# Gregor-Mendel-Institute/SNPmatch

Hardware: AMD Instinct MI355X
Metric: accession×SNP comparisons/sec (whole node); achieved HBM GB/s vs peak (higher is better)
Workload: dtype f64

## Files before the change

### snpmatch_amd/csrc/snpm_api.hip

```cpp
#include "snpmatch_hip.h"

#include <hip/hip_runtime.h>

#include <fcntl.h>
#include <unistd.h>

#include <algorithm>
#include <atomic>
#include <cerrno>
#include <cmath>
#include <cstdarg>
#include <cstdio>
#include <cstdlib>
#include <chrono>
#include <cstring>
#include <map>
#include <mutex>
#include <new>
#include <stdexcept>
#include <string>
#include <thread>
#include <vector>

#include "snpm_kernels.hpp"
// ... 148 lines not shown
    int64_t ld = 0;
    int packed = 0;
    int8_t *d = nullptr;
    int *d_other = nullptr;
    hipEvent_t uploaded = nullptr;
    bool upload_pending = false;
    hipEvent_t used = nullptr;
    bool used_valid = false;
    uint8_t *dT = nullptr;
    int64_t pitchT = 0;
    int dT_state = 0;
    std::vector<snpm_query *> queries;
};

constexpr int REEVAL_CAP = 64;

struct snpm_query {
    snpm_panel *panel = nullptr;
    int64_t n = 0, row0 = 0;
    int64_t *d_row_idx = nullptr;
    double *d_w = nullptr;
    double *d_lut = nullptr;
    int lut_skip = -1;
    double *d_score = nullptr;
    int64_t *d_ninfo = nullptr;
    double *own_score = nullptr;
    int64_t *own_ninfo = nullptr;
    double wsum = 0;
    bool all_integer = false;
    bool hard01 = false;
    uint8_t *d_wbits = nullptr;
    void *d_cert = nullptr;
    int64_t eref_chunk = -1, eref_after = -1;
    bool count_valid = false;
    bool cert_count_clean = false;
    std::vector<snpm_ctx::Cached> owned;
    const char *last_kernel = "";
    int reeval_path = 0;
    bool transient_panel = false;
    double *cert_eref() const { return (double *)d_cert; }
    int *cert_count() const { return (int *)((char *)d_cert + 8); }
    int32_t *cert_cols() const { return (int32_t *)((char *)d_cert + 16); }
};

struct snpm_carry {
    snpm_ctx *ctx = nullptr;
    int64_t n_acc = 0, ld = 0;
    double *d_score = nullptr;
    int64_t *d_ninfo = nullptr;
    double *d_E = nullptr;
    int32_t *d_cols = nullptr;
    int *d_ncols = nullptr;
    int64_t n_cols = -1;
    int64_t n_rows = 0, n_slabs = 0;
    long double wsum = 0;
    int mode = -1;
    bool all_integer = true;
    bool finished = false;
    double *own_score = nullptr;
    int64_t *own_ninfo = nullptr;
    int64_t len = 0;
};

namespace {

int set_err(snpm_ctx *ctx, int code, const char *fmt, ...)
// ... 236 lines not shown
    if (const char *s = getenv("SNPM_SHARED_TILES")) ctx->shared_force_tiles = std::max(0, atoi(s));
    if (const char *s = getenv("SNPM_KIN_WS_MB")) ctx->kin_ws_bytes = (size_t)std::max(1, atoi(s)) << 20;
    if (const char *s = getenv("SNPM_SITE_WS_MB")) ctx->site_ws_bytes = (size_t)std::max(1, atoi(s)) << 20;
    if (const char *s = getenv("SNPM_LD_WS_MB")) ctx->ld_ws_bytes = (size_t)std::max(1, atoi(s)) << 20;
    if (const char *s = getenv("SNPM_WIN_WS_MB")) ctx->win_ws_bytes = (size_t)std::max(1, atoi(s)) << 20;
    if (const char *s = getenv("SNPM_F1X_WS_MB")) ctx->f1x_ws_bytes = (size_t)std::max(1, atoi(s)) << 20;
    if (const char *s = getenv("SNPM_PAR_WS_MB")) ctx->par_ws_bytes = (size_t)std::max(1, atoi(s)) << 20;
    if (const char *s = getenv("SNPM_SIM_WS_MB")) ctx->sim_ws_bytes = (size_t)std::max(1, atoi(s)) << 20;
    if (const char *s = getenv("SNPM_MOS_WS_MB")) ctx->mos_ws_bytes = (size_t)std::max(1, atoi(s)) << 20;
    if (const char *s = getenv("SNPM_IBD_WS_MB")) ctx->ibd_ws_bytes = (size_t)std::max(1, atoi(s)) << 20;
    if (const char *s = getenv("SNPM_IBD_BITS_MB")) ctx->ibd_bits_bytes = (size_t)std::max(1, atoi(s)) << 20;
    if (const char *s = getenv("SNPM_MK_WS_MB")) ctx->mk_ws_bytes = (size_t)std::max(1, atoi(s)) << 20;
    ctx->stage_threads = default_stage_threads();
    if (const char *s = getenv("SNPM_STAGE_THREADS")) ctx->stage_threads = std::max(1, atoi(s));
    if (const char *s = getenv("SNPM_STAGE_MB")) ctx->ld_want = (size_t)std::max(1, atoi(s)) << 20;
    if (const char *s = getenv("SNPM_HOST_PACK")) ctx->host_pack = atoi(s);
    if (const char *s = getenv("SNPM_ODIRECT")) ctx->odirect = atoi(s);
    if (getenv("SNPM_NO_AVX2")) ctx->ld_avx2 = 0;
    ctx->ld_nt = (cpu_has_avx2() && ctx->ld_avx2 && !getenv("SNPM_NO_NT")) ? 1 : 0;
    *out = ctx;
    return SNPM_OK;
} SNPM_GUARD(nullptr)

static void orphan_query(snpm_query *q, bool use_hip)
{
    snpm_ctx *ctx = q->panel ? q->panel->ctx : nullptr;
    if (use_hip && ctx) {
        while (!q->owned.empty()) query_release(q, q->owned.back().p);
    } else {
        q->owned.clear();
    }
    q->d_row_idx = nullptr; q->d_w = nullptr; q->d_lut = nullptr; q->d_score = nullptr; q->d_ninfo = nullptr;
    q->own_score = nullptr; q->own_ninfo = nullptr; q->d_wbits = nullptr; q->d_cert = nullptr;
    q->panel = nullptr;
}

static void orphan_panel(snpm_panel *p, bool use_hip)
{
    for (snpm_query *q : p->queries) orphan_query(q, use_hip);
    p->queries.clear();
    if (use_hip) {
        if (p->d) (void)hipFree(p->d);
        if (p->dT) (void)hipFree(p->dT);
        if (p->uploaded) (void)hipEventDestroy(p->uploaded);
        if (p->used) (void)hipEventDestroy(p->used);
    }
    if (p->ctx && p->ctx->last_touched == p) p->ctx->last_touched = nullptr;
    p->used = nullptr;
    p->used_valid = false;
    p->d = nullptr;
    p->d_other = nullptr;
    p->dT = nullptr;
    p->uploaded = nullptr;
    p->ctx = nullptr;
}

int snpm_destroy(snpm_ctx *ctx)
{
    if (!ctx) return SNPM_OK;
    const bool use_hip = hip_alive();
    if (use_hip) {
        (void)hipSetDevice(ctx->device);
        (void)hipDeviceSynchronize();
    }
    for (snpm_group *g : ctx->groups) group_forget_ctx(g, ctx, use_hip);
    ctx->groups.clear();
// ... 144 lines not shown
```

### snpmatch_amd/csrc/snpm_api_carry.hpp

```cpp
int snpm_carry_create(snpm_ctx *ctx, int64_t n_acc, snpm_carry **out)
try {
    if (!ctx) return SNPM_ERR_BADARG;
    CHECK_ARG(ctx, out != nullptr && n_acc >= 1, "carry needs n_acc >= 1");
    HIPCHK(ctx, hipSetDevice(ctx->device));
    snpm_carry *c = new snpm_carry();
    c->ctx = ctx;
    c->n_acc = n_acc;
    c->ld = ((n_acc + 255) / 256) * 256;
    hipError_t e = hipMalloc((void **)&c->own_score, (size_t)c->ld * sizeof(double));
    if (e == hipSuccess) e = hipMalloc((void **)&c->own_ninfo, (size_t)c->ld * sizeof(int64_t));
    if (e == hipSuccess) e = hipMalloc((void **)&c->d_E, 256 + REEVAL_CAP * sizeof(int32_t));
    c->d_score = c->own_score;
    c->d_ninfo = c->own_ninfo;
    c->len = c->ld;
    if (e != hipSuccess) {
        if (c->own_score) (void)hipFree(c->own_score);
        if (c->own_ninfo) (void)hipFree(c->own_ninfo);
        delete c;
        return set_err(ctx, SNPM_ERR_OOM, "carry allocation failed: %s", hipGetErrorString(e));
    }
    c->d_ncols = (int *)((char *)c->d_E + 8);
    c->d_cols = (int32_t *)((char *)c->d_E + 256);
    ctx->carries.push_back(c);
    *out = c;
// ... 34 lines not shown
    }
    delete c;
    return SNPM_OK;
}

int snpm_carry_bind_outputs(snpm_carry *c, void *d_score, void *d_ninfo)
{
    CHECK_CARRY(c);
    snpm_ctx *ctx = c->ctx;
    CHECK_ARG(ctx, (d_score == nullptr) == (d_ninfo == nullptr), "bind both outputs or neither");
    CHECK_ARG(ctx, c->n_slabs == 0, "bind the outputs before the first slab");
    c->d_score = d_score ? (double *)d_score : c->own_score;
    c->d_ninfo = d_ninfo ? (int64_t *)d_ninfo : c->own_ninfo;
    c->len = d_score ? c->n_acc : c->ld;
    return snpm_carry_reset(c);
}

int snpm_carry_set_columns(snpm_carry *c, const int32_t *cols, int64_t ncols)
{
    CHECK_CARRY(c);
    snpm_ctx *ctx = c->ctx;
    CHECK_ARG(ctx, c->n_slabs == 0, "set the column list before the first slab");
    CHECK_ARG(ctx, ncols >= 1 && ncols <= REEVAL_CAP && cols, "a column list holds 1..64 accessions (more: a strict pass over all of them)");
    for (int64_t i = 0; i < ncols; ++i) CHECK_ARG(ctx, cols[i] >= 0 && cols[i] < c->n_acc, "accession index outside the panel");
    HIPCHK(ctx, hipSetDevice(ctx->device));
    const int nc = (int)ncols;
    HIPCHK(ctx, hipMemcpyAsync(c->d_cols, cols, (size_t)ncols * sizeof(int32_t), hipMemcpyHostToDevice, ctx->stream));
    HIPCHK(ctx, hipMemcpyAsync(c->d_ncols, &nc, sizeof(int), hipMemcpyHostToDevice, ctx->stream));
    HIPCHK(ctx, hipStreamSynchronize(ctx->stream));
    c->n_cols = ncols;
    return SNPM_OK;
}

int snpm_query_run_carry(snpm_query *q, int64_t chunk, int skip_hets, int mode, int64_t chunks_after, snpm_carry *c)
try {
    CHECK_QUERY(q);
    CHECK_CARRY(c);
    snpm_ctx *ctx = q->panel->ctx;
    snpm_panel *p = q->panel;
    CHECK_ARG(ctx, c->ctx == ctx && c->n_acc == p->n_acc, "the carry belongs to another context or panel width");
    CHECK_ARG(ctx, chunk >= 1 && chunks_after >= 0, "chunk must be >= 1 and chunks_after >= 0");
    CHECK_ARG(ctx, mode == SNPM_MODE_EXACT || mode == SNPM_MODE_STRICT || mode == SNPM_MODE_FAST, "unknown mode");
    CHECK_ARG(ctx, !c->finished, "the carry was finished: reset it first");
    CHECK_ARG(ctx, c->mode < 0 || c->mode == mode, "every slab of a job is scored in the same mode");
    CHECK_ARG(ctx, chunks_after == 0 || q->n % chunk == 0, "every slab but the last must hold a multiple of `chunk` rows");
    CHECK_ARG(ctx, c->n_cols < 0 || mode == SNPM_MODE_STRICT, "a column-list carry takes strict slabs");
    HIPCHK(ctx, hipSetDevice(ctx->device));
    int rc = wait_upload(p);
    if (rc) return rc;
    const int skip = skip_hets ? 1 : 0;
    q->transient_panel = true;
    q->count_valid = false;
    if (c->n_cols >= 0) {
        rc = run_strict_sparse(q, skip, chunk, c->d_cols, c->d_ncols, c->d_score);
        if (rc) return rc;
        HIPCHK(ctx, hipMemcpyAsync(c->d_score, ctx->ws_tmp_score.p, (size_t)c->n_cols * sizeof(double),
                                   hipMemcpyDeviceToDevice, ctx->stream));
    } else if (mode == SNPM_MODE_STRICT) {
        q->last_kernel = "k_strict4";
        rc = run_strict_chain(q, skip, chunk, nullptr, c->d_score, c->d_ninfo, c->d_score, c->d_ninfo);
        if (rc) return rc;
    } else {
        Certify cert;
        cert.on = (mode == SNPM_MODE_EXACT);
        cert.flag = false;
        cert.chunk = chunk;
        cert.chunks_after = chunks_after;
        FastGeom g;
        rc = run_fast(q, skip, &g, cert);
        if (rc) return rc;
        const bool bounded = cert.on && q->n > 0;
        if (bounded && q->all_integer) {
            rc = ensure_eref(q, chunk, chunks_after);
            if (rc) return rc;
        }
        hipLaunchKernelGGL(k_carry_add, dim3((unsigned)((p->n_acc + 255) / 256)), dim3(256), 0, ctx->stream, c->d_score,
                           c->d_ninfo, (const double *)q->d_score, (const int64_t *)q->d_ninfo, p->n_acc, c->d_E,
                           bounded ? (const double *)q->cert_eref() : (const double *)nullptr,
                           (bounded && !q->all_integer) ? efast_bound(q, g) : 0.0);
        HIPCHK(ctx, hipGetLastError());
        c->all_integer = c->all_integer && (q->all_integer || q->n == 0);
    }
    c->mode = mode;
    c->n_rows += q->n;
    c->n_slabs += 1;
    c->wsum += q->wsum;
    return SNPM_OK;
} SNPM_GUARD(((q && q->panel) ? q->panel->ctx : nullptr))

static bool carry_is_exact(const snpm_carry *c) { return c->all_integer && c->wsum < 9.0e15L; }

static double carry_e_extra(const snpm_carry *c)
{
    const double u = 1.1102230246251565e-16;
    const double m = (double)(c->n_slabs + 1);
    return (double)(c->wsum * (long double)(m * u / (1.0 - m * u))) * 1.0000001;
}

int snpm_carry_error_bound(snpm_carry *c, double *bound)
{
    CHECK_CARRY(c);
    snpm_ctx *ctx = c->ctx;
    CHECK_ARG(ctx, bound != nullptr, "bound is NULL");
    *bound = 0.0;
    if (c->mode != SNPM_MODE_EXACT || carry_is_exact(c)) return SNPM_OK;
    HIPCHK(ctx, hipSetDevice(ctx->device));
    int rc = ensure_pinned(ctx, 64);
    if (rc) return rc;
    HIPCHK(ctx, hipMemcpyAsync(ctx->h_pinned, c->d_E, sizeof(double), hipMemcpyDeviceToHost, ctx->stream));
    HIPCHK(ctx, hipStreamSynchronize(ctx->stream));
    *bound = *(const double *)ctx->h_pinned + carry_e_extra(c);
// ... 57 lines not shown
```

### snpmatch_amd/csrc/snpm_api_cert.hpp

```cpp
int ensure_pinned(snpm_ctx *ctx, size_t bytes)
{
    if (ctx->h_pinned_cap >= bytes) return SNPM_OK;
    if (ctx->h_pinned) {
        HIPCHK(ctx, hipStreamSynchronize(ctx->stream));
        (void)hipHostFree(ctx->h_pinned);
    }
    ctx->h_pinned = nullptr;
    ctx->h_pinned_cap = 0;
    const size_t want = std::max<size_t>(bytes, 64 << 10);
    HIPCHK(ctx, hipHostMalloc(&ctx->h_pinned, want, hipHostMallocDefault));
    ctx->h_pinned_cap = want;
    return SNPM_OK;
}

int ensure_eref(snpm_query *q, int64_t chunk, int64_t chunks_after)
{
    snpm_ctx *ctx = q->panel->ctx;
    if (q->eref_chunk == chunk && q->eref_after == chunks_after) return SNPM_OK;
    const int64_t K = (q->n + chunk - 1) / chunk;
    const int grid = (int)std::max<int64_t>(1, std::min<int64_t>(K, 2048));
    int rc = ensure(ctx, ctx->ws_epart, (size_t)grid * sizeof(double));
    if (rc) return rc;
    hipLaunchKernelGGL(k_eref, dim3((unsigned)grid), dim3(256), 0, ctx->stream, (const double *)q->d_w, q->n, chunk,
                       chunks_after, (double *)ctx->ws_epart.p);
    hipLaunchKernelGGL(k_efinish, dim3(1), dim3(256), 0, ctx->stream, (const double *)ctx->ws_epart.p, grid, q->n, chunk,
                       chunks_after, q->cert_eref());
    HIPCHK(ctx, hipGetLastError());
    q->eref_chunk = chunk;
    q->eref_after = chunks_after;
    return SNPM_OK;
}

double efast_bound(const snpm_query *q, const FastGeom &g)
{
    const double u = 1.1102230246251565e-16;
    const int64_t epoch_adds = (int64_t)EPOCH_TILES * (g.packed ? TILE_ROWS : std::max(g.tile_rows, TILE_ROWS));
    const double m = (double)(std::min<int64_t>(g.part_rows, epoch_adds) + REDUCE_GROUP + g.n_groups + 2);
    return (q->wsum * (m * u / (1.0 - m * u))) * 1.0000001;
}

struct Certify {
    bool on = false;
    bool flag = true;
    int64_t chunk = 1000, chunks_after = 0;
};

int fast_tile_rows(const snpm_query *q, bool bits)
{
    const snpm_panel *p = q->panel;
    if (p->packed) return bits ? BITS_TILE_ROWS : Q4_TILE_ROWS * Q4_RUN;
    const bool long_tiles = q->n >= p->ctx->long_scan_rows && p->n_acc > 2 * WAVE * 4;
    return long_tiles ? LONG_TILE_ROWS : TILE_ROWS;
}

int run_fast(snpm_query *q, int skip, FastGeom *geom_out, const Certify &cert)
{
    snpm_ctx *ctx = q->panel->ctx;
    snpm_panel *p = q->panel;
    int rc = ensure_lut(q, skip);
    if (rc) return rc;
    const bool gather = q->d_row_idx != nullptr;
    const bool p16 = p->packed != 0;
    const bool bits = p16 && q->hard01;
    const int tile_rows = fast_tile_rows(q, bits);
    const int wpb_fixed = bits ? 1 : (p16 ? q4_waves_per_block(p->n_acc) : 0);
    FastGeom g0 = fast_geom(ctx, p->n_acc, q->n, 2, p16, tile_rows, wpb_fixed);
    int occ = 0;
    const int thr = WAVE * g0.wpb;
    if (bits) (void)launch_bits(q, g0, skip, gather, &occ, thr);
    else if (p16) (void)launch_p16(q, g0, skip, gather, &occ, thr);
    else occ = occ_b(skip, gather, thr);
    const int kmult = (p16 && !bits) ? 16 : 1;
    if (gather && !p16 && g0.wpb >= 5 && g0.wpb <= 7) occ = std::min(occ, g0.wpb == 5 ? 4 : 3);
    FastGeom g = fast_geom(ctx, p->n_acc, q->n, occ, p16, tile_rows, wpb_fixed, kmult);
    if (!p16 && tile_rows == TILE_ROWS && g.n_epochs == 1 && g.n_parts > 1) {
        const int64_t n_tiles = (q->n + TILE_ROWS - 1) / TILE_ROWS;
        const int64_t k = (n_tiles + g.n_parts - 1) / g.n_parts;
        if (k <= 8 && n_tiles > g.n_parts) {
            int64_t tr = ((q->n + k * g.n_parts - 1) / (k * g.n_parts) + 7) / 8 * 8;
            tr = std::max<int64_t>(32, std::min<int64_t>(TILE_ROWS, tr));
            if (tr < TILE_ROWS) g = fast_geom(ctx, p->n_acc, q->n, occ, p16, (int)tr, wpb_fixed, kmult);
        }
    }
    if (geom_out) *geom_out = g;
    q->last_kernel = bits ? "k_fast_bits" : (p16 ? "k_fast_packed_q4" : "k_fast");
    rc = ensure(ctx, ctx->ws_part_score, (size_t)g.n_slots * p->ld * sizeof(double));
    if (rc) return rc;
    rc = ensure(ctx, ctx->ws_part_miss, (size_t)g.n_slots * p->ld * sizeof(uint32_t));
    if (rc) return rc;
    rc = ensure(ctx, ctx->ws_grp_score, (size_t)g.n_groups * p->ld * sizeof(double));
    if (rc) return rc;
    rc = ensure(ctx, ctx->ws_grp_miss, (size_t)g.n_groups * p->ld * sizeof(uint32_t));
    if (rc) return rc;
    const bool certify = cert.on && !q->all_integer && q->n > 0;
    if (certify) {
        rc = ensure_eref(q, cert.chunk, cert.chunks_after);
        if (rc) return rc;
    }
    if (!q->cert_count_clean) HIPCHK(ctx, hipMemsetAsync(q->cert_count(), 0, sizeof(int), ctx->stream));
    q->cert_count_clean = false;
    q->count_valid = cert.on;
    if (q->n > 0) {
        if (g.n_epochs > 1) {
            const size_t off = (size_t)(g.n_epochs - 1) * g.n_parts * p->ld;
            HIPCHK(ctx, hipMemsetAsync((double *)ctx->ws_part_score.p + off, 0, (size_t)g.n_parts * p->ld * sizeof(double), ctx->stream));
            HIPCHK(ctx, hipMemsetAsync((uint32_t *)ctx->ws_part_miss.p + off, 0, (size_t)g.n_parts * p->ld * sizeof(uint32_t), ctx->stream));
        }
        if (bits) rc = launch_bits(q, g, skip, gather, nullptr, thr);
        else if (p16) rc = launch_p16(q, g, skip, gather, nullptr, thr);
        else rc = launch_fast_b(q, g, skip, gather);
        if (rc) return rc;
    }
    {
        ProfScope ps(ctx, PK_REDUCE);
        const int thr = 64;
        const unsigned cb = (unsigned)((p->n_acc + thr - 1) / thr);
        const int64_t n_groups = q->n > 0 ? g.n_groups : 0;
        const double *eref = (certify && cert.flag) ? (const double *)q->cert_eref() : (const double *)nullptr;
        const double efast = certify ? efast_bound(q, g) : 0.0;
        if (n_groups > 0) {
            hipLaunchKernelGGL(k_reduce_groups, dim3(cb, (unsigned)n_groups), dim3(thr), 0, ctx->stream,
                               (const double *)ctx->ws_part_score.p, (const uint32_t *)ctx->ws_part_miss.p, g.n_slots,
                               p->ld, p->n_acc, (double *)ctx->ws_grp_score.p, (uint32_t *)ctx->ws_grp_miss.p);
            HIPCHK(ctx, hipGetLastError());
        }
        hipLaunchKernelGGL(k_reduce, dim3(cb), dim3(thr), 0, ctx->stream, (const double *)ctx->ws_grp_score.p,
                           (const uint32_t *)ctx->ws_grp_miss.p, n_groups, p->ld, p->n_acc, q->n, q->d_score,
                           q->d_ninfo, eref, efast, ctx->debug_reeval, q->cert_cols(), q->cert_count(), REEVAL_CAP);
// ... 44 lines not shown
```

### snpmatch_amd/csrc/snpm_api_launch.hpp

```cpp
struct FastGeom {
    bool packed;
    int wpb;
    int tile_rows = TILE_ROWS;
    int64_t n_wc, n_colblocks, n_parts, part_rows;
    int64_t n_epochs, n_slots, n_groups;
};

template <bool SKIP, bool GATHER>
int occupancy_of(int threads)
{
    int nb = 0;
    if (hipOccupancyMaxActiveBlocksPerMultiprocessor(&nb, k_fast<SKIP, GATHER>, threads, 0) != hipSuccess) nb = 0;
    return nb;
}

FastGeom fast_geom(snpm_ctx *ctx, int64_t n_acc, int64_t n, int occ_blocks_hint, bool packed, int tile_rows = TILE_ROWS,
                   int wpb_fixed = 0, int kernel_parts_mult = 1)
{
    FastGeom g;
    g.packed = packed;
    g.tile_rows = tile_rows;
    const int64_t span = (int64_t)WAVE * (packed ? 16 : 4);
    g.n_wc = std::max<int64_t>(1, (n_acc + span - 1) / span);
    if (wpb_fixed > 0) {
        g.wpb = (int)std::min<int64_t>(wpb_fixed, g.n_wc);
    } else if (g.n_wc <= 8) {
        g.wpb = (int)g.n_wc;
    } else {
        double best = -1.0;
        int best_w = 8;
        for (int w = 8; w >= 4; --w) {
            const int64_t blocks = (g.n_wc + w - 1) / w;
            const double active = (double)g.n_wc / (double)(blocks * w);
            const double balance = (w % 4 == 0) ? 1.0 : ((w % 2 == 0) ? 0.95 : 0.85);
            if (active * balance > best) { best = active * balance; best_w = w; }
        }
        g.wpb = best_w;
    }
    g.n_colblocks = (g.n_wc + g.wpb - 1) / g.wpb;
    int occ = occ_blocks_hint > 0 ? occ_blocks_hint : 2;
    const int64_t pitch_bytes = ((n_acc + 255) / 256) * 256;
    if (!packed && occ_blocks_hint > 0 && (g.wpb == 4 || g.wpb == 5) &&
        n * pitch_bytes >= (int64_t(32) << 30))
        occ = std::min(occ, std::max(3, 18 / g.wpb));
    if (!packed && occ_blocks_hint > 0 && g.wpb == 8 &&
        n * pitch_bytes >= (int64_t(4) << 30))
        occ = std::min(occ, 2);
    const int narrow_mult = (!packed && g.wpb == 1 && occ_blocks_hint > 0) ? 4 : 1;
    const int64_t n_tiles = std::max<int64_t>(1, (n + tile_rows - 1) / tile_rows);
    constexpr int64_t kPartMinTiles = 8;
    int kmult = 1;
    if (kernel_parts_mult > 1 && g.wpb != 5) {
        const int64_t base_parts = std::max<int64_t>(1, (int64_t)ctx->n_cu * occ * narrow_mult / g.n_colblocks);
        kmult = (int)std::max<int64_t>(1, std::min<int64_t>(kernel_parts_mult, n_tiles / (base_parts * kPartMinTiles)));
    }
    int64_t resident = (int64_t)ctx->n_cu * occ * narrow_mult * kmult;
    int64_t n_parts = std::max<int64_t>(1, resident / g.n_colblocks);
    n_parts = std::min(n_parts, n_tiles);
    if (ctx->debug_max_parts > 0) n_parts = std::min<int64_t>(n_parts, ctx->debug_max_parts);
    n_parts = std::min<int64_t>(n_parts, 65535);
    g.n_parts = n_parts;
    const int64_t tiles_per_part = (n_tiles + n_parts - 1) / n_parts;
    g.part_rows = tiles_per_part * tile_rows;
    g.n_epochs = std::max<int64_t>(1, (tiles_per_part + EPOCH_TILES - 1) / EPOCH_TILES);
    g.n_slots = g.n_epochs * g.n_parts;
    g.n_groups = (g.n_slots + REDUCE_GROUP - 1) / REDUCE_GROUP;
    return g;
}

static inline bool fast_has_pad_line(const snpm_panel *p)
{
    return p->pitch - (p->n_acc + 127) / 128 * 128 >= 128;
}

template <bool SKIP, bool GATHER, bool PAD>
int launch_fast_t(snpm_query *q, const FastGeom &g)
{
    snpm_ctx *ctx = q->panel->ctx;
    snpm_panel *p = q->panel;
    dim3 grid((unsigned)g.n_colblocks, (unsigned)g.n_parts);
    dim3 block(WAVE * g.wpb);
    ProfScope ps(ctx, PK_FAST);
    if (g.tile_rows == LONG_TILE_ROWS)
        hipLaunchKernelGGL((k_fast<SKIP, GATHER, false, LONG_TILE_ROWS, PAD>), grid, block, 0, ctx->stream, p->d,
                           p->pitch, q->d_row_idx, q->row0, q->n, q->d_lut, (double *)ctx->ws_part_score.p, (uint32_t *)ctx->ws_part_miss.p,
                           p->ld, p->n_acc, (const int64_t *)nullptr);
    else
        hipLaunchKernelGGL((k_fast<SKIP, GATHER, false, TILE_ROWS, PAD>), grid, block, 0, ctx->stream, p->d, p->pitch, q->d_row_idx, q->row0,
                           q->n, q->d_lut, (double *)ctx->ws_part_score.p, (uint32_t *)ctx->ws_part_miss.p, p->ld, p->n_acc,
                           (const int64_t *)nullptr, g.tile_rows < TILE_ROWS ? g.tile_rows : 0);
    HIPCHK(ctx, hipGetLastError());
    return SNPM_OK;
}

int launch_fast_b(snpm_query *q, const FastGeom &g, bool skip, bool gather)
{
    if (fast_has_pad_line(q->panel)) {
        if (skip)
            return gather ? launch_fast_t<true, true, true>(q, g) : launch_fast_t<true, false, true>(q, g);
        return gather ? launch_fast_t<false, true, true>(q, g) : launch_fast_t<false, false, true>(q, g);
    }
    if (skip)
        return gather ? launch_fast_t<true, true, false>(q, g) : launch_fast_t<true, false, false>(q, g);
    return gather ? launch_fast_t<false, true, false>(q, g) : launch_fast_t<false, false, false>(q, g);
}

static int q4_waves_per_block(int64_t n_acc)
{
    const int64_t n_wc = (n_acc + 1023) / 1024;
    if (n_wc <= 8) return (int)n_wc;
    int best = 4;
    int64_t best_waves = (n_wc + 3) / 4 * 4;
    for (int w : {7, 8}) {
        const int64_t waves = (n_wc + w - 1) / w * w;
        if (waves <= best_waves) {
            best = w;
            best_waves = waves;
        }
    }
    return best;
}

static int q4_tile_rows(int wpb)
{
    return wpb >= 4 ? 64 : (wpb >= 2 ? 32 : 16);
}

template <bool SKIP, bool GATHER, int TR>
int launch_p16_t(snpm_query *q, const FastGeom &g, int *occ_out, int threads)
{
    snpm_ctx *ctx = q->panel->ctx;
    snpm_panel *p = q->panel;
    if (occ_out) {
        int nb = 0;
        if (hipOccupancyMaxActiveBlocksPerMultiprocessor(&nb, k_fast_packed_q4<SKIP, GATHER, false, TR>, threads, 0) != hipSuccess) nb = 0;
        *occ_out = nb;
        return SNPM_OK;
// ... 74 lines not shown
```

### snpmatch_amd/csrc/snpm_k_fast.hpp

```cpp
#pragma once

namespace snpm {
template <int NDW, bool SKIP, int U>
__device__ __forceinline__ void fast_row(const uint32_t (&x)[NDW], uint32_t group_base, uint32_t roff4,
                                         double (&acc)[NDW * 4], uint32_t (&miss8)[NDW])
{
#ifdef SNPM_FAST_PATTERN_ONLY
#pragma unroll
    for (int k = 0; k < NDW; ++k) miss8[k] ^= x[k];
    (void)group_base; (void)roff4; (void)acc;
    return;
#endif
    double w[NDW * 4];
#pragma unroll
    for (int k = 0; k < NDW; ++k) {
        const uint32_t tix = ((x[k] << 3) & 0x18181818u) | roff4;
        if (SKIP)
            miss8[k] += ((x[k] >> 7) | ((x[k] >> 1) & ~x[k])) & 0x01010101u;
        else
            miss8[k] += (x[k] >> 7) & 0x01010101u;
#pragma unroll
        for (int j = 0; j < 4; ++j) {
            const uint32_t addr = __builtin_amdgcn_perm(tix, group_base, 0x0c0c0100u | (uint32_t)(4 + j));
            lds_cdouble *ptr = (lds_cdouble *)(uintptr_t)addr;
            w[4 * k + j] = ptr[U * 4];
        }
    }
#pragma unroll
    for (int e = 0; e < NDW * 4; ++e) acc[e] += w[e];
}

__device__ __forceinline__ void load_row(const int8_t *p, uint32_t (&x)[1])
{
    x[0] = __builtin_nontemporal_load(reinterpret_cast<const uint32_t *>(p));
}

#define SCORE_ROW(U, X, GROUP_BASE, ROFF4, ROFF) fast_row<NDW, SKIP, U>((X), (GROUP_BASE), (ROFF4), acc, miss8)

template <bool SKIP, bool GATHER, bool SEG = false, int TR = TILE_ROWS, bool PAD = false>
__global__ void __launch_bounds__(WAVE *MAX_WAVES_PER_BLOCK, SNPM_FAST_MIN_WAVES)
k_fast(const int8_t *__restrict__ db, int64_t pitch, const int64_t *__restrict__ row_idx, int64_t row0, int64_t n,
       const double *__restrict__ lut, double *__restrict__ out_score, uint32_t *__restrict__ out_miss, int64_t ld,
       int64_t n_acc, const int64_t *__restrict__ part_desc = nullptr, int tile_rows_rt = 0)
{
    constexpr int BPL = 4;
    constexpr int NDW = BPL / 4;
    constexpr int EPL = BPL;
    constexpr int G = GATHER ? SNPM_FAST_G_GATHER : SNPM_FAST_G;
    __shared__ __attribute__((aligned(256))) double s_lut[2][TR * 4];
    const int TRR = (tile_rows_rt > 0 && tile_rows_rt <= TR) ? tile_rows_rt : TR;

    const int tid = threadIdx.x;
    const int nthr = blockDim.x;
    const int64_t byte0 = ((int64_t)blockIdx.x * nthr + tid) * BPL;
    const int64_t col0 = byte0;
    const bool lane_on = byte0 < pitch && col0 < ld;
    const bool pad_lane = PAD && lane_on && byte0 >= (n_acc + 127) / 128 * 128;
    const uint32_t pad18 = pad_lane ? 0x18181818u : 0u;
    const int64_t p = SEG ? (int64_t)blockIdx.y + (int64_t)gridDim.y * blockIdx.z : (int64_t)blockIdx.y;
    if (SEG && p >= n) return;
    const int64_t rbase = SEG ? part_desc[3 * p] : 0;
    const int64_t rend = SEG ? part_desc[3 * p + 1] : n;
    const int64_t P = SEG ? 1 : (int64_t)gridDim.y;
    const int64_t T0 = SEG ? 0 : p;
    const int64_t slot0 = SEG ? part_desc[3 * p + 2] : p;
    const int64_t slot_stride = SEG ? 1 : (int64_t)gridDim.y;
    const int64_t n_tiles_total = (rend - rbase + TRR - 1) / TRR;

    double acc[EPL];
    uint32_t miss16[NDW * 2];
    uint32_t miss8[NDW];
#pragma unroll
    for (int i = 0; i < EPL; ++i) acc[i] = 0.0;
#pragma unroll
    for (int i = 0; i < NDW * 2; ++i) miss16[i] = 0;
#pragma unroll
    for (int i = 0; i < NDW; ++i) miss8[i] = 0;

    const uint32_t lane_off = !lane_on ? 0u : (pad_lane ? (uint32_t)((n_acc - 1) & ~(int64_t)3) : (uint32_t)byte0);
    auto row_ptr = [&](int64_t rr) -> const int8_t * {
        const int64_t prow = GATHER ? row_idx[rr] : (row0 + rr);
        const int8_t *rowbase = db + prow * pitch;
        uint32_t off = lane_off;
        asm volatile("" : "+v"(off));
        return rowbase + off;
    };

    auto store_partials = [&](int64_t epoch) {
        if (lane_on) {
            double *os = out_score + (slot0 + epoch * slot_stride) * ld + col0;
            uint32_t *om = out_miss + (slot0 + epoch * slot_stride) * ld + col0;
#pragma unroll
            for (int i = 0; i < EPL; i += 2) *reinterpret_cast<double2 *>(os + i) = make_double2(acc[i], acc[i + 1]);
#pragma unroll
            for (int k = 0; k < NDW; ++k) {
                uint4 m;
                m.x = miss16[2 * k + 0] & 0xffffu;
                m.y = miss16[2 * k + 1] & 0xffffu;
                m.z = miss16[2 * k + 0] >> 16;
                m.w = miss16[2 * k + 1] >> 16;
                *reinterpret_cast<uint4 *>(om + 4 * k) = m;
            }
        }
#pragma unroll
        for (int i = 0; i < EPL; ++i) acc[i] = 0.0;
#pragma unroll
        for (int i = 0; i < NDW * 2; ++i) miss16[i] = 0;
    };
    int64_t last_epoch = 0;

    if (T0 < n_tiles_total) {
        {
            const int64_t tr0 = rbase + T0 * TRR;
            const int rows2 = 2 * (int)((rend - tr0 < TRR) ? (rend - tr0) : TRR);
            const double2 *src = reinterpret_cast<const double2 *>(lut + 4 * tr0);
            double2 *dst = reinterpret_cast<double2 *>(&s_lut[0][0]);
            for (int i = tid; i < rows2; i += nthr) dst[i] = src[i];
        }
        uint32_t xa[G][NDW], xb[G][NDW];
#pragma unroll
        for (int u = 0; u < G; ++u) load_row(row_ptr(rbase + T0 * TRR + u), xa[u]);
        __syncthreads();

        int buf = 0;
        int tiles_in_epoch = 0;
        int64_t epoch = 0;
        for (int64_t T = T0; T < n_tiles_total; T += P, buf ^= 1) {
            if (tiles_in_epoch == EPOCH_TILES) {
                store_partials(epoch);
                ++epoch;
                tiles_in_epoch = 0;
            }
            ++tiles_in_epoch;
            const int64_t tr0 = rbase + T * TRR;
            const int rows = (int)((rend - tr0 < TRR) ? (rend - tr0) : TRR);
            const bool more = (T + P < n_tiles_total);
            const int64_t ntr0 = more ? rbase + (T + P) * TRR : tr0;
            double2 pre0 = make_double2(0.0, 0.0);
// ... 24 lines not shown
            SCORE_ROW(6, (X)[G > 4 ? 6 : 0], gbase_, roff4_, roff_);                        \
            SCORE_ROW(7, (X)[G > 4 ? 7 : 0], gbase_, roff4_, roff_);                        \
        }                                                                                   \
    } while (0)
            int g = 0;
            for (; g + 2 <= full_groups; g += 2) {
                const int64_t rnext = tr0 + (int64_t)(g + 1) * G;
                const int64_t rafter = (g + 2 < TRR / G) ? rnext + G : ntr0;
#pragma unroll
                for (int u = 0; u < G; ++u) load_row(row_ptr(rnext + u), xb[u]);
                SCORE_GROUP(xa, g);
#pragma unroll
                for (int u = 0; u < G; ++u) load_row(row_ptr(rafter + u), xa[u]);
                SCORE_GROUP(xb, g + 1);
            }
            if (g < full_groups) {
                SCORE_GROUP(xa, g);
            }
#undef SCORE_GROUP
            for (int r = full_groups * G; r < rows; ++r) {
                uint32_t x[NDW];
                load_row(row_ptr(tr0 + r), x);
                const uint32_t group_base = lds_base + (uint32_t)(r >> 3) * 256u;
                const uint32_t roff4 = ((uint32_t)(r & 7) * 0x20202020u) | pad18;
                SCORE_ROW(0, x, group_base, roff4, (uint32_t)(r & 7) * 32u);
            }
#pragma unroll
            for (int k = 0; k < NDW; ++k) {
                if (pad_lane) miss8[k] = (uint32_t)rows * 0x01010101u;
                miss16[2 * k + 0] += miss8[k] & 0x00ff00ffu;
                miss16[2 * k + 1] += (miss8[k] >> 8) & 0x00ff00ffu;
                miss8[k] = 0;
            }
#if !defined(SNPM_FAST_PATTERN_ONLY) || SNPM_FAST_PATTERN_ONLY != 2
            if (more) {
                double2 *dst = reinterpret_cast<double2 *>(&s_lut[buf ^ 1][0]);
                if (staged) {
                    if (tid < TRR * 2) dst[tid] = pre0;
                } else {
                    const double2 *src = reinterpret_cast<const double2 *>(lut + 4 * ntr0);
                    for (int i = tid; i < nrows2; i += nthr) dst[i] = src[i];
                }
            }
            __syncthreads();
#endif
        }
        last_epoch = epoch;
    }
    store_partials(last_epoch);
}

#undef SCORE_ROW

}
```

### snpmatch_amd/csrc/snpm_k_prep.hpp

```cpp
#pragma once

namespace snpm {
__global__ void k_build_lut(const double *__restrict__ w, double *__restrict__ lut, int64_t n, int skip_hets, int *__restrict__ bad)
{
    int64_t i = (int64_t)blockIdx.x * blockDim.x + threadIdx.x;
    if (i >= n) return;
    double w0 = w[3 * i + 0], w1 = w[3 * i + 1], w2 = w[3 * i + 2];
    if (bad && !(fabs(w0) <= 1.7976931348623157e308 && fabs(w1) <= 1.7976931348623157e308 && fabs(w2) <= 1.7976931348623157e308))
        atomicOr(bad, 4);
    double4 e;
    e.x = w0;
    e.y = w2;
    e.z = skip_hets ? 0.0 : w1;
    e.w = 0.0;
    reinterpret_cast<double4 *>(lut)[i] = e;
}

__device__ __forceinline__ double block_sum_256(double v, double *sm)
{
#pragma unroll
    for (int o = 32; o > 0; o >>= 1) v += __shfl_xor(v, o);
    const int wave = threadIdx.x >> 6;
    __syncthreads();
    if ((threadIdx.x & 63) == 0) sm[wave] = v;
// ... 29 lines not shown
    wbits[r] = b;
}

__global__ void __launch_bounds__(256)
k_eref(const double *__restrict__ w, int64_t n, int64_t chunk, int64_t chunks_after, double *__restrict__ partial)
{
    __shared__ double sm[4];
    const int64_t K = (n + chunk - 1) / chunk;
    double acc = 0.0;
    for (int64_t k = blockIdx.x; k < K; k += gridDim.x) {
        const int64_t r0 = k * chunk, r1 = (r0 + chunk < n) ? r0 + chunk : n;
        double s = 0.0;
        for (int64_t r = r0 + threadIdx.x; r < r1; r += 256)
            s += fmax(fabs(w[3 * r]), fmax(fabs(w[3 * r + 1]), fabs(w[3 * r + 2])));
        s = block_sum_256(s, sm);
        acc += s * (double)((r1 - r0) + 3 + (K - k) + chunks_after);
    }
    if (threadIdx.x == 0) partial[blockIdx.x] = acc;
}

__global__ void __launch_bounds__(256)
k_efinish(const double *__restrict__ partial, int n_partial, int64_t n, int64_t chunk, int64_t chunks_after,
          double *__restrict__ eref)
{
    __shared__ double sm[4];
    double v = 0.0;
    for (int i = threadIdx.x; i < n_partial; i += 256) v += partial[i];
    v = block_sum_256(v, sm);
    if (threadIdx.x == 0) {
        const double u = 1.1102230246251565e-16;
        const int64_t K = (n + chunk - 1) / chunk;
        const double mmax = (double)(chunk + 3 + K + chunks_after);
        eref[0] = (v * u / (1.0 - mmax * u)) * 1.0000001;
    }
}

__global__ void k_check_rows(int64_t *__restrict__ rows, const int32_t *__restrict__ src32, int64_t n, int64_t n_snp,
                             int *__restrict__ bad)
{
    const int64_t i = (int64_t)blockIdx.x * blockDim.x + threadIdx.x;
    if (i >= n) return;
    int64_t r = src32 ? (int64_t)src32[i] : rows[i];
    if (r < 0 || r >= n_snp) {
        r = 0;
        atomicOr(bad, 1);
    }
    rows[i] = r;
}

__global__ void k_expand_codes(const uint16_t *__restrict__ codes, const double *__restrict__ table, int64_t n3,
                               double *__restrict__ wei)
{
    const int64_t i = (int64_t)blockIdx.x * blockDim.x + threadIdx.x;
    if (i < n3) wei[i] = table[codes[i]];
}

constexpr int ONCE_SUB = 1024;
constexpr int64_t ONCE_MAX_CHUNK = 4096;

template <bool CODED>
__global__ void __launch_bounds__(256)
k_once_prep(const void *src_rows, const void *src_wei, const double *__restrict__ table, int table_len,
            int64_t n, int64_t n_snp, int64_t chunk, int skip_hets, int64_t *rows, double *w,
            double *__restrict__ lut, double *__restrict__ partial, double *__restrict__ eref, int *__restrict__ cert_count,
            unsigned *__restrict__ state , int pad_rows)
{
// ... 102 lines not shown
```

Baseline: 6191 billion.

## Tighten error-bound certification with chunk-sum chain and two-level fast accumulation

Replaces the per-query reference error bound in carry mode with a chain bound computed from cached per-chunk max-weight sums, evaluated by a single-block prefix-scan kernel. It adds a two-level accumulation variant of the fast kernel: per-tile partials are folded into a separate high accumulator, which shortens the rounding-error term used in efast_bound. A host-side occupancy check selects this variant only when it does not reduce occupancy. The aim is a tighter certified bound, so that fewer rows need exact re-evaluation, at the cost of extra register use and a small serial kernel per slab.

```diff
diff --git a/snpmatch_amd/csrc/snpm_api.hip b/snpmatch_amd/csrc/snpm_api.hip
--- a/snpmatch_amd/csrc/snpm_api.hip
+++ b/snpmatch_amd/csrc/snpm_api.hip
@@ -204,6 +204,8 @@
     uint8_t *d_wbits = nullptr;
     void *d_cert = nullptr;
     int64_t eref_chunk = -1, eref_after = -1;
+    double *d_csum = nullptr;
+    int64_t csum_chunk = -1;
     bool count_valid = false;
     bool cert_count_clean = false;
     std::vector<snpm_ctx::Cached> owned;
@@ -506,6 +508,7 @@
     }
     q->d_row_idx = nullptr; q->d_w = nullptr; q->d_lut = nullptr; q->d_score = nullptr; q->d_ninfo = nullptr;
     q->own_score = nullptr; q->own_ninfo = nullptr; q->d_wbits = nullptr; q->d_cert = nullptr;
+    q->d_csum = nullptr; q->csum_chunk = -1;
     q->panel = nullptr;
 }
 
diff --git a/snpmatch_amd/csrc/snpm_api_carry.hpp b/snpmatch_amd/csrc/snpm_api_carry.hpp
--- a/snpmatch_amd/csrc/snpm_api_carry.hpp
+++ b/snpmatch_amd/csrc/snpm_api_carry.hpp
@@ -90,6 +90,8 @@
     return SNPM_OK;
 }
 
+static double *carry_e_slab(const snpm_carry *c) { return (double *)((char *)c->d_E + 16); }
+
 int snpm_query_run_carry(snpm_query *q, int64_t chunk, int skip_hets, int mode, int64_t chunks_after, snpm_carry *c)
 try {
     CHECK_QUERY(q);
@@ -128,13 +130,13 @@
         rc = run_fast(q, skip, &g, cert);
         if (rc) return rc;
         const bool bounded = cert.on && q->n > 0;
-        if (bounded && q->all_integer) {
-            rc = ensure_eref(q, chunk, chunks_after);
+        if (bounded) {
+            rc = run_echain(q, chunk, (double)(c->wsum * 1.0000001L), carry_e_slab(c));
             if (rc) return rc;
         }
         hipLaunchKernelGGL(k_carry_add, dim3((unsigned)((p->n_acc + 255) / 256)), dim3(256), 0, ctx->stream, c->d_score,
                            c->d_ninfo, (const double *)q->d_score, (const int64_t *)q->d_ninfo, p->n_acc, c->d_E,
-                           bounded ? (const double *)q->cert_eref() : (const double *)nullptr,
+                           bounded ? (const double *)carry_e_slab(c) : (const double *)nullptr,
                            (bounded && !q->all_integer) ? efast_bound(q, g) : 0.0);
         HIPCHK(ctx, hipGetLastError());
         c->all_integer = c->all_integer && (q->all_integer || q->n == 0);
diff --git a/snpmatch_amd/csrc/snpm_api_cert.hpp b/snpmatch_amd/csrc/snpm_api_cert.hpp
--- a/snpmatch_amd/csrc/snpm_api_cert.hpp
+++ b/snpmatch_amd/csrc/snpm_api_cert.hpp
@@ -31,11 +31,39 @@
     return SNPM_OK;
 }
 
+int run_echain(snpm_query *q, int64_t chunk, double w_before, double *e_slab)
+{
+    snpm_ctx *ctx = q->panel->ctx;
+    const int64_t K = (q->n + chunk - 1) / chunk;
+    if (q->csum_chunk != chunk) {
+        if (q->d_csum) query_release(q, q->d_csum);
+        q->d_csum = nullptr;
+        q->csum_chunk = -1;
+        if (query_alloc(q, (void **)&q->d_csum, (size_t)K * sizeof(double)) != hipSuccess) {
+            (void)hipGetLastError();
+            q->d_csum = nullptr;
+            return set_err(ctx, SNPM_ERR_OOM, "no memory for the chunk sums of the error bound");
+        }
+        const int grid = (int)std::max<int64_t>(1, std::min<int64_t>(K, 2048));
+        hipLaunchKernelGGL(k_chunk_sums, dim3((unsigned)grid), dim3(256), 0, ctx->stream, (const double *)q->d_w, q->n, chunk,
+                           q->d_csum);
+        HIPCHK(ctx, hipGetLastError());
+        q->csum_chunk = chunk;
+    }
+    hipLaunchKernelGGL(k_echain, dim3(1), dim3(ECHAIN_THREADS), 0, ctx->stream, (const double *)q->d_csum, q->n, chunk, w_before, e_slab);
+    HIPCHK(ctx, hipGetLastError());
+    return SNPM_OK;
+}
+
 double efast_bound(const snpm_query *q, const FastGeom &g)
 {
     const double u = 1.1102230246251565e-16;
     const int64_t epoch_adds = (int64_t)EPOCH_TILES * (g.packed ? TILE_ROWS : std::max(g.tile_rows, TILE_ROWS));
-    const double m = (double)(std::min<int64_t>(g.part_rows, epoch_adds) + REDUCE_GROUP + g.n_groups + 2);
+    int64_t part_adds = std::min<int64_t>(g.part_rows, epoch_adds);
+    if (g.two_level && !g.packed)
+        part_adds = std::min<int64_t>(part_adds, std::min<int64_t>(g.part_rows, g.tile_rows) +
+                                                     std::min<int64_t>(g.part_rows / g.tile_rows, EPOCH_TILES));
+    const double m = (double)(part_adds + REDUCE_GROUP + g.n_groups + 2);
     return (q->wsum * (m * u / (1.0 - m * u))) * 1.0000001;
 }
 
@@ -82,6 +110,7 @@
             if (tr < TILE_ROWS) g = fast_geom(ctx, p->n_acc, q->n, occ, p16, (int)tr, wpb_fixed, kmult);
         }
     }
+    g.two_level = fast_two_level(ctx, p, g, skip != 0, gather);
     if (geom_out) *geom_out = g;
     q->last_kernel = bits ? "k_fast_bits" : (p16 ? "k_fast_packed_q4" : "k_fast");
     rc = ensure(ctx, ctx->ws_part_score, (size_t)g.n_slots * p->ld * sizeof(double));
@@ -93,7 +122,7 @@
     rc = ensure(ctx, ctx->ws_grp_miss, (size_t)g.n_groups * p->ld * sizeof(uint32_t));
     if (rc) return rc;
     const bool certify = cert.on && !q->all_integer && q->n > 0;
-    if (certify) {
+    if (certify && cert.flag) {
         rc = ensure_eref(q, cert.chunk, cert.chunks_after);
         if (rc) return rc;
     }
diff --git a/snpmatch_amd/csrc/snpm_api_launch.hpp b/snpmatch_amd/csrc/snpm_api_launch.hpp
--- a/snpmatch_amd/csrc/snpm_api_launch.hpp
+++ b/snpmatch_amd/csrc/snpm_api_launch.hpp
@@ -4,6 +4,8 @@
     int tile_rows = TILE_ROWS;
     int64_t n_wc, n_colblocks, n_parts, part_rows;
     int64_t n_epochs, n_slots, n_groups;
+    int occ = 0;
+    bool two_level = false;
 };
 
 template <bool SKIP, bool GATHER>
@@ -60,6 +62,7 @@
     if (ctx->debug_max_parts > 0) n_parts = std::min<int64_t>(n_parts, ctx->debug_max_parts);
     n_parts = std::min<int64_t>(n_parts, 65535);
     g.n_parts = n_parts;
+    g.occ = occ * narrow_mult * kmult;
     const int64_t tiles_per_part = (n_tiles + n_parts - 1) / n_parts;
     g.part_rows = tiles_per_part * tile_rows;
     g.n_epochs = std::max<int64_t>(1, (tiles_per_part + EPOCH_TILES - 1) / EPOCH_TILES);
@@ -81,6 +84,17 @@
     dim3 grid((unsigned)g.n_colblocks, (unsigned)g.n_parts);
     dim3 block(WAVE * g.wpb);
     ProfScope ps(ctx, PK_FAST);
+    if constexpr (!GATHER) {
+        if (g.two_level) {
+            if (g.tile_rows != LONG_TILE_ROWS) return set_err(ctx, SNPM_ERR_STATE, "two-level sums need long tiles");
+            hipLaunchKernelGGL((k_fast<SKIP, false, false, LONG_TILE_ROWS, PAD, true>), grid, block, 0, ctx->stream, p->d,
+                               p->pitch, q->d_row_idx, q->row0, q->n, q->d_lut, (double *)ctx->ws_part_score.p,
+                               (uint32_t *)ctx->ws_part_miss.p, p->ld, p->n_acc, (const int64_t *)nullptr);
+            HIPCHK(ctx, hipGetLastError());
+            return SNPM_OK;
+        }
+    }
+    if (g.two_level) return set_err(ctx, SNPM_ERR_STATE, "two-level sums on a gathered launch");
     if (g.tile_rows == LONG_TILE_ROWS)
         hipLaunchKernelGGL((k_fast<SKIP, GATHER, false, LONG_TILE_ROWS, PAD>), grid, block, 0, ctx->stream, p->d,
                            p->pitch, q->d_row_idx, q->row0, q->n, q->d_lut, (double *)ctx->ws_part_score.p, (uint32_t *)ctx->ws_part_miss.p,
@@ -103,6 +117,30 @@
     if (skip)
         return gather ? launch_fast_t<true, true, false>(q, g) : launch_fast_t<true, false, false>(q, g);
     return gather ? launch_fast_t<false, true, false>(q, g) : launch_fast_t<false, false, false>(q, g);
+}
+
+static bool fast_two_level(const snpm_ctx *ctx, const snpm_panel *p, const FastGeom &g, bool skip, bool gather)
+{
+    if (g.packed || gather || g.tile_rows != LONG_TILE_ROWS) return false;
+    static int occ_cache[2][2][MAX_WAVES_PER_BLOCK + 1];
+    const bool pad = fast_has_pad_line(p);
+    int &c = occ_cache[skip ? 1 : 0][pad ? 1 : 0][g.wpb];
+    if (c == 0) {
+        int nb = 0;
+        hipError_t e;
+        const int thr = WAVE * g.wpb;
+        if (skip)
+            e = pad ? hipOccupancyMaxActiveBlocksPerMultiprocessor(&nb, k_fast<true, false, false, LONG_TILE_ROWS, true, true>, thr, 0)
+                    : hipOccupancyMaxActiveBlocksPerMultiprocessor(&nb, k_fast<true, false, false, LONG_TILE_ROWS, false, true>, thr, 0);
+        else
+            e = pad ? hipOccupancyMaxActiveBlocksPerMultiprocessor(&nb, k_fast<false, false, false, LONG_TILE_ROWS, true, true>, thr, 0)
+                    : hipOccupancyMaxActiveBlocksPerMultiprocessor(&nb, k_fast<false, false, false, LONG_TILE_ROWS, false, true>, thr, 0);
+        if (e != hipSuccess) (void)hipGetLastError();
+        c = (e == hipSuccess && nb > 0) ? nb : -1;
+    }
+    const int64_t blocks = g.n_parts * g.n_colblocks;
+    const int64_t per_cu = std::min<int64_t>(g.occ, (blocks + ctx->n_cu - 1) / std::max(1, ctx->n_cu));
+    return c >= per_cu && per_cu * g.wpb <= 4 * SNPM_FAST_MIN_WAVES;
 }
 
 static int q4_waves_per_block(int64_t n_acc)
diff --git a/snpmatch_amd/csrc/snpm_k_fast.hpp b/snpmatch_amd/csrc/snpm_k_fast.hpp
--- a/snpmatch_amd/csrc/snpm_k_fast.hpp
+++ b/snpmatch_amd/csrc/snpm_k_fast.hpp
@@ -37,12 +37,13 @@
 
 #define SCORE_ROW(U, X, GROUP_BASE, ROFF4, ROFF) fast_row<NDW, SKIP, U>((X), (GROUP_BASE), (ROFF4), acc, miss8)
 
-template <bool SKIP, bool GATHER, bool SEG = false, int TR = TILE_ROWS, bool PAD = false>
+template <bool SKIP, bool GATHER, bool SEG = false, int TR = TILE_ROWS, bool PAD = false, bool TWO = false>
 __global__ void __launch_bounds__(WAVE *MAX_WAVES_PER_BLOCK, SNPM_FAST_MIN_WAVES)
 k_fast(const int8_t *__restrict__ db, int64_t pitch, const int64_t *__restrict__ row_idx, int64_t row0, int64_t n,
        const double *__restrict__ lut, double *__restrict__ out_score, uint32_t *__restrict__ out_miss, int64_t ld,
        int64_t n_acc, const int64_t *__restrict__ part_desc = nullptr, int tile_rows_rt = 0)
 {
+    static_assert(!TWO || (!GATHER && !SEG && TR == LONG_TILE_ROWS), "two-level sums: dense long-tile launches only");
     constexpr int BPL = 4;
     constexpr int NDW = BPL / 4;
     constexpr int EPL = BPL;
@@ -68,10 +69,13 @@
     const int64_t n_tiles_total = (rend - rbase + TRR - 1) / TRR;
 
     double acc[EPL];
+    double hi[TWO ? EPL : 1];
     uint32_t miss16[NDW * 2];
     uint32_t miss8[NDW];
 #pragma unroll
     for (int i = 0; i < EPL; ++i) acc[i] = 0.0;
+#pragma unroll
+    for (int i = 0; i < (TWO ? EPL : 1); ++i) hi[i] = 0.0;
 #pragma unroll
     for (int i = 0; i < NDW * 2; ++i) miss16[i] = 0;
 #pragma unroll
@@ -91,7 +95,10 @@
             double *os = out_score + (slot0 + epoch * slot_stride) * ld + col0;
             uint32_t *om = out_miss + (slot0 + epoch * slot_stride) * ld + col0;
 #pragma unroll
-            for (int i = 0; i < EPL; i += 2) *reinterpret_cast<double2 *>(os + i) = make_double2(acc[i], acc[i + 1]);
+            for (int i = 0; i < EPL; i += 2) {
+                if constexpr (TWO) *reinterpret_cast<double2 *>(os + i) = make_double2(hi[i], hi[i + 1]);
+                else *reinterpret_cast<double2 *>(os + i) = make_double2(acc[i], acc[i + 1]);
+            }
 #pragma unroll
             for (int k = 0; k < NDW; ++k) {
                 uint4 m;
@@ -104,6 +111,10 @@
         }
 #pragma unroll
         for (int i = 0; i < EPL; ++i) acc[i] = 0.0;
+        if constexpr (TWO) {
+#pragma unroll
+            for (int i = 0; i < EPL; ++i) hi[i] = 0.0;
+        }
 #pragma unroll
         for (int i = 0; i < NDW * 2; ++i) miss16[i] = 0;
     };
@@ -194,6 +205,13 @@
                 miss16[2 * k + 1] += (miss8[k] >> 8) & 0x00ff00ffu;
                 miss8[k] = 0;
             }
+            if constexpr (TWO) {
+#pragma unroll
+                for (int i = 0; i < EPL; ++i) {
+                    hi[i] += acc[i];
+                    acc[i] = 0.0;
+                }
+            }
 #if !defined(SNPM_FAST_PATTERN_ONLY) || SNPM_FAST_PATTERN_ONLY != 2
             if (more) {
                 double2 *dst = reinterpret_cast<double2 *>(&s_lut[buf ^ 1][0]);
diff --git a/snpmatch_amd/csrc/snpm_k_prep.hpp b/snpmatch_amd/csrc/snpm_k_prep.hpp
--- a/snpmatch_amd/csrc/snpm_k_prep.hpp
+++ b/snpmatch_amd/csrc/snpm_k_prep.hpp
@@ -85,6 +85,97 @@
         const int64_t K = (n + chunk - 1) / chunk;
         const double mmax = (double)(chunk + 3 + K + chunks_after);
         eref[0] = (v * u / (1.0 - mmax * u)) * 1.0000001;
+    }
+}
+
+__global__ void __launch_bounds__(256)
+k_chunk_sums(const double *__restrict__ w, int64_t n, int64_t chunk, double *__restrict__ csum)
+{
+    __shared__ double sm[4];
+    const int64_t K = (n + chunk - 1) / chunk;
+    for (int64_t k = blockIdx.x; k < K; k += gridDim.x) {
+        const int64_t r0 = k * chunk, r1 = (r0 + chunk < n) ? r0 + chunk : n;
+        double s = 0.0;
+        for (int64_t r = r0 + threadIdx.x; r < r1; r += 256)
+            s += fmax(fabs(w[3 * r]), fmax(fabs(w[3 * r + 1]), fabs(w[3 * r + 2])));
+        s = block_sum_256(s, sm);
+        if (threadIdx.x == 0) csum[k] = s;
+    }
+}
+
+__device__ __forceinline__ double pow2_floor(double x)
+{
+    return __longlong_as_double(__double_as_longlong(x) & 0x7ff0000000000000ll);
+}
+
+constexpr int ECHAIN_THREADS = 1024;
+constexpr int ECHAIN_BATCH = 8;
+
+__global__ void __launch_bounds__(ECHAIN_THREADS)
+k_echain(const double *__restrict__ csum, int64_t n, int64_t chunk, double w_before, double *__restrict__ e_slab)
+{
+    constexpr int NW = ECHAIN_THREADS / 64, NB = ECHAIN_BATCH;
+    __shared__ double s_wave[NW], s_in[NW], s_ch[NW];
+    const int64_t K = (n + chunk - 1) / chunk;
+    const int64_t L = (K + ECHAIN_THREADS - 1) / ECHAIN_THREADS;
+    const int t = threadIdx.x, lane = t & 63, wave = t >> 6;
+    const int64_t k0 = (int64_t)t * L < K ? (int64_t)t * L : K;
+    const int64_t k1 = k0 + L < K ? k0 + L : K;
+    double mine = 0.0;
+    for (int64_t k = k0; k < k1; k += NB) {
+        double v[NB];
+#pragma unroll
+        for (int j = 0; j < NB; ++j) v[j] = (k + j < k1) ? csum[k + j] : 0.0;
+#pragma unroll
+        for (int j = 0; j < NB; ++j) mine += v[j];
+    }
+    double incl = mine;
+#pragma unroll
+    for (int o = 1; o < 64; o <<= 1) {
+        const double v = __shfl_up(incl, o);
+        if (lane >= o) incl += v;
+    }
+    if (lane == 63) s_wave[wave] = incl;
+    double excl = __shfl_up(incl, 1);
+    if (lane == 0) excl = 0.0;
+    __syncthreads();
+    double before = w_before;
+    for (int wv = 0; wv < wave; ++wv) before += s_wave[wv];
+    double run = before + excl;
+    double in_chunk = 0.0, chain = 0.0;
+    for (int64_t k = k0; k < k1; k += NB) {
+        double v[NB];
+#pragma unroll
+        for (int j = 0; j < NB; ++j) v[j] = (k + j < k1) ? csum[k + j] : 0.0;
+#pragma unroll
+        for (int j = 0; j < NB; ++j) {
+            if (k + j < k1) {
+                const int64_t len = (k + j == K - 1) ? n - (K - 1) * chunk : chunk;
+                in_chunk += v[j] * (double)(len + 3);
+                run += v[j];
+                chain += pow2_floor(run * 1.0000001);
+            }
+        }
+    }
+#pragma unroll
+    for (int o = 32; o > 0; o >>= 1) {
+        in_chunk += __shfl_xor(in_chunk, o);
+        chain += __shfl_xor(chain, o);
+    }
+    if (lane == 0) {
+        s_in[wave] = in_chunk;
+        s_ch[wave] = chain;
+    }
+    __syncthreads();
+    if (t == 0) {
+        double a = 0.0, c = 0.0;
+        for (int wv = 0; wv < NW; ++wv) {
+            a += s_in[wv];
+            c += s_ch[wv];
+        }
+        const double u = 1.1102230246251565e-16;
+        const double mmax = (double)(chunk + 3);
+        e_slab[0] = (a * u / (1.0 - mmax * u) + c * u) * 1.0000001;
     }
 }
 
```

Result: faster. 6256 billion (median of 6 runs) (+1.0%).
